# pierrepaleo/PDWT

Hardware: AMD Instinct MI355X
Metric: Mpixels/s fwd+inv DWT (4096² db4 L3) (higher is better)
Workload: dtype f32; 1 GPU; 4096x4096 float32, db4, 3 levels, separable DWT fwd+inv (BASELINE.json configs[1]); levels=3, parallelism=batch-split x1 (no data-path collective)

## Files before the change

### pdwt_amd/csrc/casc_dev.hpp

```cpp
#pragma once
#include "common.hpp"

#ifndef PDWT_CASC_DIAG
#define PDWT_CASC_DIAG 0
#endif
#define CASC_DIAG_ST(row) ((PDWT_CASC_DIAG & 1) ? ((row) & 31) : (row))
#define CASC_DIAG_LD(row) ((PDWT_CASC_DIAG & 2) ? ((row) & 31) : (row))

namespace pdwt {

template <int HLEN>
struct CascGeom {
    static constexpr int C = HLEN / 2 - 1;
    static constexpr int NB1 = C > 0 ? (C + 3) / 4 : 0;
    static constexpr int NB2 = C > 0 ? (C + 1) / 2 : 0;
    static constexpr int NBT = NB1 + NB2;
    static constexpr int WIN1 = 4 * (2 * NB1 + 1);
    static constexpr int WIN2 = 2 * (2 * NB2 + 1);
    static constexpr int MAXVL = 64 - 2 * NBT;
};

struct CascMap {
    int cpx;
    int strips;
// ... 4 lines not shown
__host__ __device__ inline int casc_chunk_start(int g, int strip, int units, int gy, int strips, int cpx, int d)
{
    if (g >= gy) return units;
    int b = (int)(((long long)g * units) / gy);
    if (d != 0) {
        int bal = 0;
        for (int q = 0; q < g; q++) bal += (((q * strips + strip) / cpx) & 1) ? -1 : 1;
        b += d * bal;
    }
    return b;
}

struct CascBands {
    float *H1, *V1, *D1, *A2, *H2, *V2, *D2;
};
struct CascBatchF {
    const float* in;
    CascBands b;
};

template <int HLEN>
struct CascInvGeom {
    static constexpr int H2 = HLEN / 2;
    static constexpr int C = H2 / 2;
    static constexpr int SHIFT = (H2 & 1) ? 0 : 1;
    static constexpr int NB1 = C > 0 ? (C + 1) / 2 : 0;
    static constexpr int NB2 = C;
    static constexpr int NBT = NB1 + NB2;
    static constexpr int WIN1 = 2 * (2 * NB1 + 1);
    static constexpr int WIN2 = 2 * NB2 + 1;
// ... 45 lines not shown
```

### pdwt_amd/csrc/common.hpp

```cpp
#pragma once
#include <atomic>
#include <hip/hip_runtime.h>
#include <hip/hip_ext.h>
#include <stddef.h>
#include <stdint.h>

#include "../../include/pdwt_hip.h"

namespace pdwt {

void set_last_error(hipError_t e, const char* what, const char* file, int line);

#define PDWT_HIP_TRY(expr)                                              \
    do {                                                                \
        hipError_t _e = (expr);                                         \
        if (_e != hipSuccess) {                                         \
            ::pdwt::set_last_error(_e, #expr, __FILE__, __LINE__);      \
            return PDWT_EHIP;                                           \
        }                                                               \
    } while (0)

hipStream_t stream();

enum KernelId {
// ... 126 lines not shown
    KN_F64_LDS_SKEW,
    KN_NORM2SQ_REF1D,
    KN_NORM_IN_THRESHOLD,
    KN_SELFCHECK,
    KN_DWT1D_F64,
    KN_SWTF_LONG,
    KN_F64_TAIL,
    KN_EXP0,
    KN_EXP1,
    KN_EXP2,
    KN_EXP3,
    KN_NONSEP_TILED,
    KN_F64_LAT,
    KN_F64_LAT_MIN,
    KN_DWT1D_NT_MB,
    KN_COUNT
};
int knob(KnobId id);
bool counted_waits_ok();
void stat_casc_spec(int inverse);
enum StatId {
    ST_INV_CASC3,
    ST_INV_CASCW,
    ST_INV_CASC2,
    ST_FWD1D_FUSED,
    ST_INV1D_FUSED,
    ST_FWD1D_FUSED_IP,
    ST_INV1D_FUSED_IP,
    ST_ANA_ROWS_TR,
    ST_SYN_ROWS_TR,
    ST_ANA_COLS_RING,
    ST_SYN_COLS_RING,
    ST_SWT_ANA_ROWS_LDS,
    ST_SWT_SYN_ROWS_LDS,
    ST_SWT_ANA_COLS_RING,
    ST_SWT_SYN_COLS_RING,
    ST_SWTF_FWD,
    ST_SWTF_INV,
    ST_SWTF_INVP,
    ST_SWTL2_FWD,
    ST_SWTL2_INV,
    ST_SWTD_FWD,
    ST_SWTD_INV,
    ST_COUNT
};
void stat_hit(StatId id);
int knob_set(const char* name, int value);
int knob_get(const char* name, int* value);

__host__ __device__ inline int div2(int n) { return (n + 1) >> 1; }
inline int idiv_up(int a, int b) { return (a + b - 1) / b; }

__device__ __forceinline__ int wrap_ext(int s, int n)
{
    const int np = n + (n & 1);
    if ((unsigned)s >= (unsigned)np) {
        s %= np;
        if (s < 0) s += np;
// ... 50 lines not shown
```

### pdwt_amd/csrc/dwt.hip

```cpp
#include <stdlib.h>
#include <string.h>

#include "common.hpp"
#include "cols_ring.hpp"
#include "rows_tr.hpp"
#include "dwt1d_fused.hpp"
#include <new>
#include <vector>

#include "dwt_lds.hpp"
#include "dwt_lat.hpp"
#include "dwt_stream.hpp"
#include "dwt_casc.hpp"
#include "casc_dev.hpp"

namespace pdwt {

constexpr int kThreads = 256;

template <typename T, int HLEN, int TX, int TY>
__global__ __launch_bounds__(kThreads) void k_fwd2d_fused(const T* __restrict__ in, T* __restrict__ cA, T* __restrict__ cH,
                                                           T* __restrict__ cV, T* __restrict__ cD, int Nr, int Nc, int hlen_rt,
                                                           Taps2<T> f)
{
// ... 589 lines not shown
template <typename T>
static int forward_separable(T* d_image, T** c, T* d_tmp, pdwt_info w, const typename FiltersOf<T>::type* filt)
{
    int rc = check_args(d_image, c, d_tmp, w, 2, true, filt, filt ? filt->hlen : 0);
    if (rc != PDWT_OK) return rc;
    const Taps2<T> f = taps_fwd<T>(filt);
    Scratch<T> s(d_tmp, w.Nr, w.Nc, 2);
    const T* in = d_image;
    int nr = w.Nr, nc = w.Nc;
    int pp = 0;
    for (int lev = 0; lev < w.nlevels; lev++) {
        if constexpr (sizeof(T) == 4) {
            if (lev + 1 < w.nlevels && !force_twopass()) {
                T* a2 = (lev + 2 == w.nlevels) ? c[0] : s.ping[pp];
                float* trash = s.t1_is_trash ? (float*)s.t1 : nullptr;
                rc = fwd2d_casc_f32(in, c[3 * lev + 1], c[3 * lev + 2], c[3 * lev + 3], a2, c[3 * lev + 4], c[3 * lev + 5], c[3 * lev + 6],
                                    trash, nr, nc, w.hlen, f);
                if (rc < 0) return rc;
                if (rc == PDWT_OK) {
                    in = a2;
                    pp ^= 1;
                    nr = div2(div2(nr));
                    nc = div2(div2(nc));
                    lev++;
                    continue;
                }
            }
        }
        T* aout = (lev == w.nlevels - 1) ? c[0] : s.ping[pp];
        rc = level_fwd2d(in, aout, c[3 * lev + 1], c[3 * lev + 2], c[3 * lev + 3], s.t1, s.t2, s.trash_floats, nr, nc, w.hlen, f,
                         d_tmp + pdwt_tmp_elems(w) - 256);
        if (rc != PDWT_OK) return rc;
        in = aout;
// ... 562 lines not shown
```

### pdwt_amd/csrc/dwt_casc.hip

```cpp
#include "dwt_casc.hpp"

#include <algorithm>

#include "dwt_stream.hpp"
#include "stream_dev.hpp"
#include "casc_dev.hpp"

namespace pdwt {

constexpr int casc_fwd_stores(int p) { return 3 + 4 * (p & 1); }
template <int DIST>
constexpr int casc_fwd_after(int p)
{
    int n = casc_fwd_stores(p);
    for (int k = 1; k < DIST; k++) n += 2 + casc_fwd_stores(p + k);
    return n;
}

template <int HLEN>
constexpr int casc_fwd_region_bytes() { return (HLEN - 2) * 64 * (16 + 8); }

#define PDWT_VB_F0 " op_sel_hi:[0,1,0]"
#define PDWT_VB_N0 " op_sel_hi:[0,1,1]"
#define PDWT_VB_F1 " op_sel:[1,0,0] op_sel_hi:[1,1,0]"
// ... 49 lines not shown
template <int HLEN, int R2, bool LV, int DIST>
struct CascSpec {
    static constexpr int NA = 2 * R2, NA1 = NA + HLEN - 2, NL1 = NA - HLEN / 2 + 1;
    static constexpr int LIM = LV ? NA1 : NL1;
    static constexpr int stores_at(int q) { return ((q < NA) ? 3 : 0) + (((q & 1) && q >= HLEN - 1) ? 4 : 0); }
    static constexpr int loads_at(int q) { return (q < LIM && q + DIST < LIM) ? 2 : 0; }
    static constexpr int wait_cnt(int n)
    {
        const int m = n - DIST;
        int c = stores_at(m);
        for (int k = 1; k < DIST; k++) c += loads_at(m + k) + stores_at(m + k);
        return c;
    }
};

template <int HLEN, int NV, int W, bool SPEC = false>
__global__ __launch_bounds__(W == 1 ? 256 : 64 * W) void k_fwd2d_casc(const float* in, CascBands b, int Nr, int Nc, int VL,
                                                                       float* __restrict__ trash, CascMap cm, TapsLH f)
{
    using G = CascGeom<HLEN>;
    constexpr int C = G::C, NB1 = G::NB1, NB2 = G::NB2, NBT = G::NBT, WIN1 = G::WIN1, WIN2 = G::WIN2;
    extern __shared__ __attribute__((aligned(16))) unsigned char lds_raw[];
    CASC_TRACE_DECL;
    CASC_TRACE(0);
    if constexpr (W > 1) {
        if (cm.tbl) {
            static_assert(sizeof(CascBatchF) == 8 * sizeof(void*), "eight pointers per image");
            typedef const unsigned long long __attribute__((address_space(4))) * tbl_t;
            const tbl_t q = (tbl_t)(const unsigned long long*)cm.tbl + 8 * (size_t)blockIdx.y;
            in = (const float*)q[0];
            b = CascBands{(float*)q[1], (float*)q[2], (float*)q[3], (float*)q[4], (float*)q[5], (float*)q[6], (float*)q[7]};
        }
    }
// ... 139 lines not shown
            }
            lplast = p1;
        } else {
            p0 = p1 = lplast;
        }
        lr += 2;
    };
    unsigned s1off = (unsigned)wrap1(2 * j0 - C, Nr2) * (unsigned)Nc2 * 4u;
    const unsigned s1end = (unsigned)Nr2 * (unsigned)Nc2 * 4u;
    unsigned s2off = (unsigned)j0 * (unsigned)Nc4 * 4u;
    (void)trash;
    const int hand_sb = __builtin_amdgcn_readfirstlane((W > 1 && kw > 0) ? 0 : -1);
    CASC_TRACE(1);
    static_for<NV>([&](auto K) { asm_drain1(v[decltype(K)::value]); });
    CASC_TRACE(2);
    auto a1_row = [&](auto A, int sb) {
            constexpr int a = decltype(A)::value;
            constexpr int u = a % (HLEN / 2);
            constexpr int s0 = (2 * u + HLEN - 2) % HLEN, s1 = (2 * u + HLEN - 1) % HLEN;
            const int n = sb * HLEN + a;
            constexpr int r0 = (2 * a) % NV, r1 = r0 + 1;
            int nq1 = n, nq2 = n;
            asm("" : "+s"(nq1));
            asm("" : "+s"(nq2));
            if (nq2 < lim2) {
                if (nq1 < lim1) {
                    asm_wait2<casc_fwd_after<DIST>((a + HLEN - DIST) % HLEN)>(v[r0], v[r1]);
                    row_pass1(v[r0], ring[s0]);
                    row_pass1(v[r1], ring[s1]);
                } else {
// ... 36 lines not shown
                    if (sb == hand_sb) *lds_ring2(lds_wr, a) = ring2[a];
                }
            } else {
                if constexpr (W > 1) ring2[a] = *lds_ring2(lds_rd, min(n - NA, HLEN - 3));
            }
            if constexpr (a & 1) {
                v2f ah2 = {0.f, 0.f}, vd2 = {0.f, 0.f};
                static_for<HLEN>([&](auto J) {
                    constexpr int j = decltype(J)::value;
                    constexpr int s = (a + 1 + j) % HLEN;
                    const v2f t = f.t[HLEN - 1 - j];
                    ah2 = pk_fma(splat(ring2[s].x), t, ah2);
                    vd2 = pk_fma(splat(ring2[s].y), t, vd2);
                });
                const bool own = (unsigned)(n - (HLEN - 1)) < (unsigned)(2 * rows2);
                asm_store4_sm(b.A2, b.H2, b.V2, b.D2, off2 + s2off, ah2.x, ah2.y, vd2.x, vd2.y, own ? vmask : 0ull);
                s2off += own ? (unsigned)Nc4 * 4u : 0u;
            }
    };
    auto epilogue = [&]() __attribute__((always_inline)) {
        CASC_TRACE(5);
#ifdef PDWT_CASC_TRACE
        asm volatile("s_waitcnt vmcnt(0)" ::: "memory");
#endif
        CASC_TRACE(6);
        CASC_TRACE_STORE(trash, blockIdx.x * W + kw, ((unsigned long long)NA1 << 32) | (unsigned)rows2);
    };
    if constexpr (SPEC) {
        static_assert(W == 16 && (NV == 2 || NV == 4), "wave programs exist for the 16-wave workgroups");
        const unsigned xoff_odd = xoff + (unsigned)strideB;
        auto spec = [&](auto R2c, auto LASTc) __attribute__((always_inline)) {
            constexpr int R2 = decltype(R2c)::value;
            constexpr bool LV = decltype(LASTc)::value;
            using S = CascSpec<HLEN, R2, LV, DIST>;
            constexpr int sNA = S::NA, sNA1 = S::NA1, sNL1 = S::NL1;
            constexpr int WR = LV ? 4 * R2 + 3 * C : 3 * C;
// ... 72 lines not shown
                if constexpr ((n & 1) && n >= HLEN - 1) {
                    v2f ah2 = {0.f, 0.f}, vd2 = {0.f, 0.f};
                    if constexpr (HLEN == 8) {
                        constexpr int q = (a + 1) % 8;
                        col_pass8x1(ah2, vd2, ring2[q], ring2[(q + 1) % 8], ring2[(q + 2) % 8], ring2[(q + 3) % 8], ring2[(q + 4) % 8], ring2[(q + 5) % 8],
                                    ring2[(q + 6) % 8], ring2[(q + 7) % 8], f.t[7], f.t[6], f.t[5], f.t[4], f.t[3], f.t[2], f.t[1], f.t[0]);
                    } else {
                        static_for<HLEN>([&](auto J) {
                            constexpr int j = decltype(J)::value;
                            constexpr int s = (a + 1 + j) % HLEN;
                            const v2f t = f.t[HLEN - 1 - j];
                            ah2 = pk_fma_vbcast<0, j == 0>(ring2[s], t, ah2);
                            vd2 = pk_fma_vbcast<1, j == 0>(ring2[s], t, vd2);
                        });
                    }
                    asm_store4_sm(b.A2, b.H2, b.V2, b.D2, off2 + s2off, ah2.x, ah2.y, vd2.x, vd2.y, vmask);
                    s2off += (unsigned)Nc4 * 4u;
                }
                if constexpr (n == HLEN / 2 - 1 || n == HLEN - 1) asm volatile("s_waitcnt lgkmcnt(0)\n\ts_barrier" ::: "memory");

#ifdef PDWT_CASC_TRACE
                if constexpr (n == HLEN / 2 - 1) CASC_TRACE(3);
                if constexpr (n == HLEN - 1) CASC_TRACE(4);
#endif
            });
        };
        const int variant = __builtin_amdgcn_readfirstlane(last ? 3 : (rows2 == 5 ? 2 : 1));
        if (variant == 1) {
            spec(std::integral_constant<int, 4>{}, std::false_type{});
            epilogue();
            __builtin_amdgcn_endpgm();
// ... 15 lines not shown
        if (sb == 0) CASC_TRACE(3);
#endif
        if (sb * HLEN + HLEN / 2 >= NA1) break;
        static_for<HLEN / 2>([&](auto U) { a1_row(std::integral_constant<int, decltype(U)::value + HLEN / 2>{}, sb); });
        if constexpr (W > 1) {
            if (sb == 0) asm volatile("s_waitcnt lgkmcnt(0)\n\ts_barrier" ::: "memory");
        }
#ifdef PDWT_CASC_TRACE
        if (sb == 0) CASC_TRACE(4);
#endif
        if (sb * HLEN + HLEN >= NA1) break;
    }
    static_for<NV>([&](auto K) { asm_drain1(v[decltype(K)::value]); });
    epilogue();
    }
}

template <int HLEN, int PFD>
__global__ __launch_bounds__(256) void k_inv2d_casc(CascInvBands b, float* __restrict__ out, int Nr, int Nc, int VL,
                                                     float* __restrict__ trash, CascMap cm, Taps2<float> f)
{
    using G = CascInvGeom<HLEN>;
    constexpr int H2 = G::H2, C = G::C, SHIFT = G::SHIFT, NB1 = G::NB1, NB2 = G::NB2, NBT = G::NBT, WIN1 = G::WIN1, WIN2 = G::WIN2;
    constexpr int VM_PF = PFD * (4 + 2 * (3 + 2));
    static_assert(VM_PF - 3 <= 63, "vmcnt is a 6-bit counter");
    static_assert(H2 % PFD == 0 || PFD % H2 == 0, "register slots must be compile-time constants");
    const int lane = threadIdx.x & 63;
    const int xcd = blockIdx.x & 7;
    const int wi = (blockIdx.x >> 3) * 4 + __builtin_amdgcn_readfirstlane(threadIdx.x >> 6);
    if (wi >= cm.cpx * cm.strips) return;
// ... 242 lines not shown
        asm_drain1(q2[k][2]);
        asm_drain1(q2[k][3]);
    });
    static_for<2 * PFD>([&](auto K) {
        constexpr int k = decltype(K)::value;
        asm_drain1(q1[k][0]);
        asm_drain1(q1[k][1]);
        asm_drain1(q1[k][2]);
    });
}

#define PDWT_CHECK_LAUNCH() PDWT_HIP_TRY(hipGetLastError())

static bool casc_enabled() { return knob(KN_CASC) == 1; }

template <int HLEN>
static int launch_fwd_casc(const float* in, const CascBands& b, float* trash, int nr, int nc, const Taps2<float>& f2, const CascBatchF* d_tbl, int nimg)
{
    TapsLH f;
    for (int k = 0; k < PDWT_MAX_FILTER_WIDTH; k++) f.t[k] = v2f{f2.a[k], f2.b[k]};
    constexpr int MAXVL = CascGeom<HLEN>::MAXVL;
    const int strips = idiv_up(nc, MAXVL * 4);
    const int VL = idiv_up(nc / 4, strips);
    constexpr int NVD = HLEN > 16 ? 4 : (HLEN % 4 == 0 ? HLEN / 2 : HLEN);
    KTimer kt(K_FWD2D_CASC, true);
    int W = knob(KN_CASC_WG);
    if (W == 0) W = 16;
    if (W != 1 && W != 4 && W != 8 && W != 16) W = 16;
    constexpr size_t REG = casc_fwd_region_bytes<HLEN>();
    while (W > 1 && (size_t)(W - 1) * REG > 150 * 1024) W /= 2;
    if (W == 2) W = 1;
    if (W > 1) {
        const int nr4 = nr / 4;
        const int wgs = knob(KN_CASC_WAVES) > 0 ? idiv_up(knob(KN_CASC_WAVES), W) : 256;
        int gy = std::max(1, wgs / strips);
        while (W > 4 && (nr4 / gy) / W < HLEN / 2) W /= 2;
        while (gy > 1 && (nr4 / gy) / W < HLEN / 2) gy--;
        if (gy >= 1 && (nr4 / gy) / W >= HLEN / 2) {
            int nwg = gy * strips;
            const size_t lds = (size_t)(W - 1) * REG;
            void (*k)(const float*, CascBands, int, int, int, float*, CascMap, TapsLH);
            k = (W == 4) ? k_fwd2d_casc<HLEN, NVD, 4> : (W == 8) ? k_fwd2d_casc<HLEN, NVD, 8> : k_fwd2d_casc<HLEN, NVD, 16>;
            const bool nv2 = W == 16 && (knob(KN_CASC_NV) == 0 || knob(KN_CASC_NV) == 2);
            if (nv2) k = k_fwd2d_casc<HLEN, 2, 16>;
            bool spec = nv2 && (knob(KN_CASC_SPEC) & 1) && 2 * 4 >= HLEN;
            auto spec_ok = [&](int gyq, int xwq) {
                const int cpxq = idiv_up(gyq * strips, 8);
                for (int g = 0; g < gyq; g++)
                    for (int st = 0; st < strips; st++) {
                        const int R = casc_chunk_start(g + 1, st, nr4, gyq, strips, cpxq, xwq) - casc_chunk_start(g, st, nr4, gyq, strips, cpxq, xwq);
                        if (R < 16) return false;
                        const int E = std::min((3 * (HLEN - 2) + 3) / 4, R / 16 - 1);
                        const int base = (R + E) / 16, rem = (R + E) % 16;
                        if (base != 4 || R - (15 * base + std::min(15, rem)) != 1) return false;
                    }
                return true;
            };
            if (spec && (knob(KN_CASC_SPEC) & 4) && knob(KN_CASC_WAVES) <= 0 && !d_tbl && (nr4 / gy) / 16 >= 8) {
                const int gy2 = (nr4 + 36) / 73;
                if (gy2 >= 3 * gy && spec_ok(gy2, 0)) {
                    gy = gy2;
                    nwg = gy * strips;
                }
            }
            int xw = spec ? knob(KN_CASC_XCDW) : 0;
            if (spec && xw != 0 && !spec_ok(gy, xw)) xw = 0;
            spec = spec && spec_ok(gy, xw);
            if (!spec) xw = 0;
            if (spec) {
                k = k_fwd2d_casc<HLEN, 2, 16, true>;
                stat_casc_spec(0);
            }
            const CascMap cm = {idiv_up(nwg, 8), strips, gy, xw, d_tbl};
            const dim3 grid((unsigned)(8 * cm.cpx), (unsigned)(d_tbl ? nimg : 1));
            if (lds > 64 * 1024) {
                int rc = (W == 4) ? lds_opt_in<k_fwd2d_casc<HLEN, NVD, 4>>()
                         : (W == 8) ? lds_opt_in<k_fwd2d_casc<HLEN, NVD, 8>>() : lds_opt_in<k_fwd2d_casc<HLEN, NVD, 16>>();
                if (rc == PDWT_OK && nv2) rc = lds_opt_in<k_fwd2d_casc<HLEN, 2, 16>>();
                if (rc == PDWT_OK && spec) rc = lds_opt_in<k_fwd2d_casc<HLEN, 2, 16, true>>();
                if (rc != PDWT_OK) return rc;
            }
            PDWT_LAUNCH_KT(kt, k, grid, dim3(64 * W), lds, in, b, nr, nc, VL, trash, cm, f);
            PDWT_CHECK_LAUNCH();
            return PDWT_OK;
        }
    }
    if (d_tbl) return 1;
    int cpx = (knob(KN_CASC_WAVES) > 0 ? knob(KN_CASC_WAVES) : 1024) / (8 * strips);
    if (cpx > nr / 4 / 4 / 8) cpx = nr / 4 / 4 / 8;
    if (cpx < 1) cpx = 1;
    const CascMap cm = {cpx, strips, 0};
    const dim3 grid((unsigned)(8 * idiv_up(cpx * strips, 4)));
    const int nv = knob(KN_CASC_NV) > 0 ? knob(KN_CASC_NV) : NVD;
    if (nv == 2)
        PDWT_LAUNCH_KT(kt, (k_fwd2d_casc<HLEN, 2, 1>), grid, dim3(256), 0, in, b, nr, nc, VL, trash, cm, f);
    else if (nv < HLEN && HLEN % 4 == 0)
        PDWT_LAUNCH_KT(kt, (k_fwd2d_casc<HLEN, NVD, 1>), grid, dim3(256), 0, in, b, nr, nc, VL, trash, cm, f);
    else
        PDWT_LAUNCH_KT(kt, (k_fwd2d_casc<HLEN, (HLEN > 16 ? NVD : HLEN), 1>), grid, dim3(256), 0, in, b, nr, nc, VL, trash, cm, f);
    PDWT_CHECK_LAUNCH();
    return PDWT_OK;
}

#ifdef PDWT_CASC_ONLY8
#define PDWT_CASC_FWD_HLENS(X) X(8)
#else
#define PDWT_CASC_FWD_HLENS(X) X(4) X(6) X(8) X(10) X(12) X(14) X(16) X(18) X(20)
#endif

int fwd2d_casc_f32(const float* in, float* H1, float* V1, float* D1, float* A2, float* H2, float* V2, float* D2, float* trash, int nr,
                   int nc, int hlen, const Taps2<float>& f, const CascBatchF* d_tbl, int nimg)
{
    if (!casc_enabled() || !stream_enabled() || !trash) return 1;
    if ((nr & 3) || (nc & 3) || nc < 256 || nr < 16 * hlen) return 1;
    if ((long long)nr * nc < (long long)knob(KN_CASC_MIN)) return 1;
    if ((long long)nr * nc >= (1LL << 32)) return 1;
    if (!al16(in) || !al16(H1) || !al16(V1) || !al16(D1) || !al16(A2) || !al16(H2) || !al16(V2) || !al16(D2)) return 1;
    const CascBands b = {H1, V1, D1, A2, H2, V2, D2};
    switch (hlen) {
#define X(H) \
    case H: return launch_fwd_casc<H>(in, b, trash, nr, nc, f, d_tbl, nimg);
        PDWT_CASC_FWD_HLENS(X)
#undef X
        default: return 1;
    }
}

template <int HLEN>
static int launch_inv_casc(const CascInvBands& b, float* out, float* trash, int nr, int nc, const Taps2<float>& f)
{
    constexpr int MAXVL = CascInvGeom<HLEN>::MAXVL;
    const int nc1 = nc / 2;
    const int strips = idiv_up(nc1, MAXVL * 2);
    const int VL = idiv_up(nc1 / 2, strips);
    int cpx = (knob(KN_CASC_IWAVES) > 0 ? knob(KN_CASC_IWAVES) : 2048) / (8 * strips);
    if (cpx > nr / 2 / 8 / 8) cpx = nr / 2 / 8 / 8;
// ... 50 lines not shown
```

### pdwt_amd/csrc/dwt_casc.hpp

```cpp
#pragma once
#include "common.hpp"
#include "casc_dev.hpp"

namespace pdwt {
int fwd2d_casc_f32(const float* in, float* H1, float* V1, float* D1, float* A2, float* H2, float* V2, float* D2, float* trash, int nr,
                   int nc, int hlen, const Taps2<float>& f, const CascBatchF* d_tbl = nullptr, int nimg = 1);
int inv2d_casc_f32(const float* A2, const float* H2, const float* V2, const float* D2, const float* H1, const float* V1, const float* D1,
                   float* out, float* trash, int nr, int nc, int hlen, const Taps2<float>& f);
}
```

### pdwt_amd/csrc/runtime.hip

```cpp
#include <set>
#include <utility>
#include <stdio.h>
#include <stdlib.h>
#include <string.h>

#include <mutex>
#include <vector>

#include "common.hpp"

namespace pdwt {

static thread_local char g_err[512] = "";

void set_last_error(hipError_t e, const char* what, const char* file, int line)
{
    snprintf(g_err, sizeof(g_err), "%s: %s (%s:%d)", hipGetErrorString(e), what, file, line);
    (void)hipGetLastError();
}

static std::mutex g_mu;
static hipStream_t g_streams[64] = {};
static hipStream_t g_user_streams[64] = {};
static bool g_user_set[64] = {};
// ... 30 lines not shown
static const KnobDef g_knob_defs[KN_COUNT] = {
    {"force_twopass", "PDWT_FORCE_TWOPASS", 0}, {"tiled_cols", "PDWT_TILED_COLS", 0},
    {"casc", "PDWT_CASC", 1}, {"casc_waves", "PDWT_CASC_WAVES", 0}, {"casc_nv", "PDWT_CASC_NV", 0},
    {"casc_min", "PDWT_CASC_MIN", 2048 * 2048}, {"casc_iwaves", "PDWT_CASC_IWAVES", 0}, {"casc_ipfd", "PDWT_CASC_IPFD", 1},
    {"casc_wg", "PDWT_CASC_WG", 0}, {"casc_iwg", "PDWT_CASC_IWG", 0}, {"casc_l3", "PDWT_CASC_L3", 1}, {"casc_spec", "PDWT_CASC_SPEC", 7}, {"casc_xcdw", "PDWT_CASC_XCDW", 0}, {"dwt1d_lds_kb", "PDWT_DWT1D_LDS_KB", 80},
    {"stream", "PDWT_STREAM", 1}, {"stream_r", "PDWT_STREAM_R", 0}, {"stream_waves", "PDWT_STREAM_WAVES", 8192},
    {"stream_narrow", "PDWT_STREAM_NARROW", 2048 * 2048}, {"small", "PDWT_SMALL", 1},
    {"rows_tr", "PDWT_ROWS_TR", 1}, {"ring_r", "PDWT_RING_R", 0}, {"ring_waves", "PDWT_RING_WAVES", 4096},
    {"swtf", "PDWT_SWTF", 1}, {"swtf_m", "PDWT_SWTF_M", 0}, {"swtf_mi", "PDWT_SWTF_MI", 0},
    {"swtf_xcd", "PDWT_SWTF_XCD", 1}, {"swtf_alt", "PDWT_SWTF_ALT", 1}, {"swtf_perm", "PDWT_SWTF_PERM", 1}, {"swtf_f64", "PDWT_SWTF_F64", 1},
    {"f64_lds", "PDWT_F64_LDS", 1}, {"f64_lds_min", "PDWT_F64_LDS_MIN", 256}, {"f64_lds_wgs", "PDWT_F64_LDS_WGS", 512}, {"f64_lds_mingroups", "PDWT_F64_LDS_MINGROUPS", 1}, {"f64_lds_skew", "PDWT_F64_LDS_SKEW", 64}, {"norm2sq_ref1d", "PDWT_NORM2SQ_REF1D", 0},
    {"norm_in_threshold", "PDWT_NORM_IN_THRESHOLD", -1},
    {"selfcheck", "PDWT_SELFCHECK", 1}, {"dwt1d_f64", "PDWT_DWT1D_F64", 1}, {"swtf_long", "PDWT_SWTF_LONG", 1}, {"f64_tail", "PDWT_F64_TAIL", 0},
    {"exp0", "PDWT_EXP0", 0}, {"exp1", "PDWT_EXP1", 0}, {"exp2", "PDWT_EXP2", 0}, {"exp3", "PDWT_EXP3", 0}, {"nonsep_tiled", "PDWT_NONSEP_TILED", 1},
    {"f64_lat", "PDWT_F64_LAT", 1}, {"f64_lat_min", "PDWT_F64_LAT_MIN", 4096}, {"dwt1d_nt_mb", "PDWT_DWT1D_NT_MB", 192},
};
static int g_knob_vals[KN_COUNT];
static std::once_flag g_knob_once;
static void knob_init()
{
    for (int i = 0; i < KN_COUNT; i++) {
        const char* e = getenv(g_knob_defs[i].env);
        g_knob_vals[i] = (e && *e) ? atoi(e) : g_knob_defs[i].dflt;
    }
}
int knob(KnobId id)
{
    std::call_once(g_knob_once, knob_init);
    return g_knob_vals[id];
}
// ... 5 lines not shown
        if (!strcmp(name, g_knob_defs[i].name)) {
            g_knob_vals[i] = value;
            return PDWT_OK;
        }
    }
    return PDWT_EINVAL;
}

std::atomic<int> g_stat_spec_fwd{0}, g_stat_spec_inv{0};
void stat_casc_spec(int inverse) { (inverse ? g_stat_spec_inv : g_stat_spec_fwd).fetch_add(1, std::memory_order_relaxed); }
std::atomic<int> g_stat_lat_fwd{0}, g_stat_lat_inv{0};
void stat_lat(int inverse) { (inverse ? g_stat_lat_inv : g_stat_lat_fwd).fetch_add(1, std::memory_order_relaxed); }
static const char* const g_stat_names[ST_COUNT] = {
    "inv_casc3", "inv_cascw", "inv_casc2", "fwd1d_fused", "inv1d_fused", "fwd1d_fused_ip", "inv1d_fused_ip", "ana_rows_tr", "syn_rows_tr",
    "ana_cols_ring", "syn_cols_ring", "swt_ana_rows_lds", "swt_syn_rows_lds", "swt_ana_cols_ring", "swt_syn_cols_ring",
    "swtf_fwd", "swtf_inv", "swtf_invp", "swtl2_fwd", "swtl2_inv", "swtd_fwd", "swtd_inv",
};
static std::atomic<int> g_stat_hits[ST_COUNT];
void stat_hit(StatId id) { g_stat_hits[id].fetch_add(1, std::memory_order_relaxed); }

int knob_get(const char* name, int* value)
{
    std::call_once(g_knob_once, knob_init);
    if (!name || !value) return PDWT_EINVAL;
    if (!strcmp(name, "stat_casc_spec_fwd") || !strcmp(name, "stat_casc_spec_inv")) {
        *value = (name[15] == 'f' ? g_stat_spec_fwd : g_stat_spec_inv).load(std::memory_order_relaxed);
        return PDWT_OK;
    }
    if (!strcmp(name, "stat_lat_fwd") || !strcmp(name, "stat_lat_inv")) {
        *value = (name[9] == 'f' ? g_stat_lat_fwd : g_stat_lat_inv).load(std::memory_order_relaxed);
        return PDWT_OK;
// ... 205 lines not shown
{
    float ms = -1.f;
    if (hipEventElapsedTime(&ms, (hipEvent_t)a, (hipEvent_t)b) != hipSuccess) return -1.f;
    return ms;
}
int pdwt_event_destroy(void* ev)
{
    PDWT_HIP_TRY(hipEventDestroy((hipEvent_t)ev));
    return PDWT_OK;
}

int pdwt_graph_allowed(void) { return (g_kt_on || g_probe_on) ? 0 : 1; }
int pdwt_graph_capture_begin(void)
{
    (void)pdwt::counted_waits_ok();
    PDWT_HIP_TRY(hipStreamBeginCapture(pdwt::stream(), hipStreamCaptureModeThreadLocal));
    return PDWT_OK;
}
int pdwt_graph_capture_end(void** exec_out)
{
    if (!exec_out) return PDWT_EINVAL;
    *exec_out = nullptr;
    hipGraph_t g = nullptr;
    hipError_t e = hipStreamEndCapture(pdwt::stream(), &g);
    if (e != hipSuccess || !g) {
        (void)hipGetLastError();
        return PDWT_EHIP;
    }
    hipGraphExec_t x = nullptr;
    e = hipGraphInstantiate(&x, g, nullptr, nullptr, 0);
// ... 130 lines not shown
```

### pdwt_amd/csrc/stream_dev.hpp

```cpp
#pragma once
#include <stdlib.h>

#include <type_traits>

#include "common.hpp"

#if defined(__HIP_DEVICE_COMPILE__) && !defined(__gfx950__)
#error "pdwt_amd streaming kernels: gfx950 (MI355X) only -- see stream_dev.hpp"
#endif

namespace pdwt {

__device__ __forceinline__ float dpp_shr1(float src)
{
    return __int_as_float(__builtin_amdgcn_mov_dpp(__float_as_int(src), 0x138, 0xf, 0xf, true));
}
__device__ __forceinline__ float dpp_shl1(float src)
{
    return __int_as_float(__builtin_amdgcn_mov_dpp(__float_as_int(src), 0x130, 0xf, 0xf, true));
}

__device__ __forceinline__ int wrapi(int s, int n)
{
    s %= n;
// ... 116 lines not shown
    asm volatile("s_and_saveexec_b64 %0, %4\n\tglobal_store_dwordx4 %1, %2, %3\n\ts_nop 1\n\ts_mov_b64 exec, %0"
                 : "=&s"(saved) : "v"(voff), "v"(d), "s"(sbase), "s"(mask) : "memory", "scc");
}
__device__ __forceinline__ void asm_store3_sm(float* b0, float* b1, float* b2, unsigned voff, v2f d0, v2f d1, v2f d2, lanemask_t mask)
{
    lanemask_t saved;
    asm volatile("s_and_saveexec_b64 %0, %8\n\tglobal_store_dwordx2 %1, %2, %5\n\tglobal_store_dwordx2 %1, %3, %6\n\tglobal_store_dwordx2 %1, %4, %7\n\ts_mov_b64 exec, %0"
                 : "=&s"(saved) : "v"(voff), "v"(d0), "v"(d1), "v"(d2), "s"(b0), "s"(b1), "s"(b2), "s"(mask) : "memory", "scc");
}
__device__ __forceinline__ void asm_store4_sm(float* b0, float* b1, float* b2, float* b3, unsigned voff, float d0, float d1, float d2, float d3, lanemask_t mask)
{
    lanemask_t saved;
    asm volatile("s_and_saveexec_b64 %0, %10\n\tglobal_store_dword %1, %2, %6\n\tglobal_store_dword %1, %3, %7\n\tglobal_store_dword %1, %4, %8\n\tglobal_store_dword %1, %5, %9\n\ts_mov_b64 exec, %0"
                 : "=&s"(saved) : "v"(voff), "v"(d0), "v"(d1), "v"(d2), "v"(d3), "s"(b0), "s"(b1), "s"(b2), "s"(b3), "s"(mask) : "memory", "scc");
}
__device__ __forceinline__ void asm_store_sm_nt(float* sbase, unsigned voff, v4f d, lanemask_t mask)
{
    lanemask_t saved;
    asm volatile("s_and_saveexec_b64 %0, %4\n\tglobal_store_dwordx4 %1, %2, %3 nt\n\ts_nop 1\n\ts_mov_b64 exec, %0"
                 : "=&s"(saved) : "v"(voff), "v"(d), "s"(sbase), "s"(mask) : "memory", "scc");
}
__device__ __forceinline__ float asm_copy(const float& src)
{
    float d;
    asm volatile("v_mov_b32 %0, %1" : "=v"(d) : "v"(src));
    return d;
}
__device__ __forceinline__ v2f asm_copy(const v2f& src)
{
    v2f d;
// ... 38 lines not shown
```

Baseline: 344,200 Mpixels/s.

## Fold third DWT level into cascaded forward kernel via tile completion counters

When the forward cascade kernel produces the second-to-last level, each workgroup now bumps atomic counters for its neighbouring tiles, and the last contributor for a tile computes the third level (A3/H3/V3/D3) from the freshly written A2 in LDS. This removes the separate level-3 kernel launch and the re-read pass over A2. In exchange it adds atomics, acquire fences, extra LDS per workgroup (which may reduce occupancy), and tail work done serially by the last workgroup of each neighbourhood.

```diff
diff --git a/pdwt_amd/csrc/casc_dev.hpp b/pdwt_amd/csrc/casc_dev.hpp
--- a/pdwt_amd/csrc/casc_dev.hpp
+++ b/pdwt_amd/csrc/casc_dev.hpp
@@ -42,6 +42,21 @@
 struct CascBands {
     float *H1, *V1, *D1, *A2, *H2, *V2, *D2;
 };
+struct CascFl3 {
+    float *A3, *H3, *V3, *D3;
+    unsigned* cnt;
+    int need;
+    int flags;
+};
+__host__ __device__ inline int casc_fl3_ring(int n) { return n < 3 ? n : 3; }
+__host__ __device__ inline int casc_fl3_first(int a0) { return (a0 + 1) >> 1; }
+constexpr int kFl3LdsHead = 64 * sizeof(int);
+__host__ __device__ inline size_t casc_fl3_lds(int oy, int ox, int hlen)
+{
+    const size_t ri = 2 * (size_t)oy + hlen - 2, ci = 2 * (size_t)ox + hlen - 2;
+    return kFl3LdsHead + sizeof(float) * (ri * ci + 2 * ri * (size_t)ox);
+}
+
 struct CascBatchF {
     const float* in;
     CascBands b;
diff --git a/pdwt_amd/csrc/common.hpp b/pdwt_amd/csrc/common.hpp
--- a/pdwt_amd/csrc/common.hpp
+++ b/pdwt_amd/csrc/common.hpp
@@ -164,11 +164,13 @@
     KN_F64_LAT,
     KN_F64_LAT_MIN,
     KN_DWT1D_NT_MB,
+    KN_CASC_FL3,
     KN_COUNT
 };
 int knob(KnobId id);
 bool counted_waits_ok();
 void stat_casc_spec(int inverse);
+unsigned* casc_fl3_counters();
 enum StatId {
     ST_INV_CASC3,
     ST_INV_CASCW,
@@ -192,6 +194,7 @@
     ST_SWTL2_INV,
     ST_SWTD_FWD,
     ST_SWTD_INV,
+    ST_CASC_FL3,
     ST_COUNT
 };
 void stat_hit(StatId id);
diff --git a/pdwt_amd/csrc/dwt.hip b/pdwt_amd/csrc/dwt.hip
--- a/pdwt_amd/csrc/dwt.hip
+++ b/pdwt_amd/csrc/dwt.hip
@@ -627,9 +627,13 @@
             if (lev + 1 < w.nlevels && !force_twopass()) {
                 T* a2 = (lev + 2 == w.nlevels) ? c[0] : s.ping[pp];
                 float* trash = s.t1_is_trash ? (float*)s.t1 : nullptr;
+                const bool tail = (lev + 3 == w.nlevels);
+                const CascL3Out b3 = {c[0], tail ? c[3 * lev + 7] : nullptr, tail ? c[3 * lev + 8] : nullptr, tail ? c[3 * lev + 9] : nullptr};
+                bool folded = false;
                 rc = fwd2d_casc_f32(in, c[3 * lev + 1], c[3 * lev + 2], c[3 * lev + 3], a2, c[3 * lev + 4], c[3 * lev + 5], c[3 * lev + 6],
-                                    trash, nr, nc, w.hlen, f);
+                                    trash, nr, nc, w.hlen, f, nullptr, 1, tail ? &b3 : nullptr, &folded);
                 if (rc < 0) return rc;
+                if (rc == PDWT_OK && folded) return PDWT_OK;
                 if (rc == PDWT_OK) {
                     in = a2;
                     pp ^= 1;
diff --git a/pdwt_amd/csrc/dwt_casc.hip b/pdwt_amd/csrc/dwt_casc.hip
--- a/pdwt_amd/csrc/dwt_casc.hip
+++ b/pdwt_amd/csrc/dwt_casc.hip
@@ -1,6 +1,8 @@
 #include "dwt_casc.hpp"
 
 #include <algorithm>
+#include <cstddef>
+#include <mutex>
 
 #include "dwt_stream.hpp"
 #include "stream_dev.hpp"
@@ -87,9 +89,119 @@
     }
 };
 
-template <int HLEN, int NV, int W, bool SPEC = false>
-__global__ __launch_bounds__(W == 1 ? 256 : 64 * W) void k_fwd2d_casc(const float* in, CascBands b, int Nr, int Nc, int VL,
-                                                                       float* __restrict__ trash, CascMap cm, TapsLH f)
+struct CascFwdArgs {
+    const float* in;
+    CascBands b;
+    int Nr, Nc, VL;
+    float* trash;
+    CascMap cm;
+    TapsLH f;
+    CascFl3 fl;
+};
+static_assert(offsetof(CascFwdArgs, b) == 8 && offsetof(CascFwdArgs, Nr) == 64 && offsetof(CascFwdArgs, trash) == 80 && offsetof(CascFwdArgs, cm) == 88 &&
+                  offsetof(CascFwdArgs, f) == 112 && offsetof(CascFwdArgs, fl) == 112 + sizeof(TapsLH) && sizeof(CascFl3) == 48,
+              "the argument offsets in the code object's metadata (llvm-readelf --notes) for k_fwd2d_casc_l3");
+typedef const CascFwdArgs __attribute__((address_space(4))) * casc_fwd_args_t;
+template <int HLEN, int W>
+__device__ __forceinline__ void casc_fl3_finish(unsigned char* lds)
+{
+    constexpr int C = HLEN / 2 - 1;
+    casc_fwd_args_t ka = (casc_fwd_args_t)__builtin_amdgcn_kernarg_segment_ptr();
+    asm volatile("" : "+s"(ka));
+    unsigned* const cnt = ka->fl.cnt;
+    if (!cnt) return;
+    asm volatile("s_waitcnt vmcnt(0) lgkmcnt(0)\n\ts_barrier" ::: "memory");
+    const int lane = threadIdx.x & 63, kw = __builtin_amdgcn_readfirstlane(threadIdx.x >> 6);
+    const CascMap cm = {ka->cm.cpx, ka->cm.strips, ka->cm.gy, ka->cm.flags, nullptr};
+    const int VL = ka->VL, Nr4 = ka->Nr >> 2, Nc4 = ka->Nc >> 2;
+    const float* const A2 = ka->b.A2;
+    const int xflags = ka->fl.flags;
+    const struct { float *A3, *H3, *V3, *D3; int need; } fl = {ka->fl.A3, ka->fl.H3, ka->fl.V3, ka->fl.D3, ka->fl.need};
+    struct { v2f t[HLEN]; } f;
+#pragma unroll
+    for (int j = 0; j < HLEN; j++) f.t[j] = ka->f.t[j];
+    const int wg = (blockIdx.x & 7) * cm.cpx + (blockIdx.x >> 3);
+    const int wgy = wg / cm.strips, strip = wg - wgy * cm.strips;
+    int* const flag = reinterpret_cast<int*>(lds);
+    if (kw == 0) {
+        const int r = min(lane / 3, 2), c = lane % 3;
+        const bool on = lane < 9 && r < casc_fl3_ring(cm.gy) && c < casc_fl3_ring(cm.strips);
+        const int tile = wrap1(wgy + r - 1, cm.gy) * cm.strips + wrap1(strip + c - 1, cm.strips);
+        const unsigned got = asm_ticket_sm(cnt, (unsigned)tile * 4u, __ballot(on));
+        const bool mine = on && got + 1u == (unsigned)fl.need;
+        asm_store_sm_wt(cnt, (unsigned)tile * 4u, 0u, __ballot(mine));
+        flag[lane] = mine ? tile : -1;
+    }
+    __syncthreads();
+    const int Nc8 = Nc4 >> 1;
+    float* const win = reinterpret_cast<float*>(lds + kFl3LdsHead);
+    for (int k = 0; k < 9; k++) {
+        const int tile = __builtin_amdgcn_readfirstlane(flag[k]);
+        if (tile < 0 || (xflags & 2)) continue;
+        if (!(xflags & 1)) __builtin_amdgcn_fence(__ATOMIC_ACQUIRE, "agent");
+        const int tg = tile / cm.strips, ts = tile - tg * cm.strips;
+        const int J0 = casc_chunk_start(tg, ts, Nr4, cm.gy, cm.strips, cm.cpx, cm.flags);
+        const int J1 = casc_chunk_start(tg + 1, ts, Nr4, cm.gy, cm.strips, cm.cpx, cm.flags);
+        const int X0 = ts * VL, X1 = min(X0 + VL, Nc4);
+        const int oy0 = casc_fl3_first(J0), OY = casc_fl3_first(J1) - oy0, ox0 = casc_fl3_first(X0), OX = casc_fl3_first(X1) - ox0;
+        const int RI = 2 * OY + HLEN - 2, CI = 2 * OX + HLEN - 2;
+        float* const rb = win + RI * CI;
+        {
+            const int gy0 = 2 * oy0 - C, gx0 = 2 * ox0 - C;
+            const int c0 = min(lane, CI - 1), c1 = min(lane + 64, CI - 1);
+            const int gc0 = wrapi(gx0 + c0, Nc4), gc1 = wrapi(gx0 + c1, Nc4);
+            for (int r = kw; r < RI; r += 4 * W) {
+                float v0[4], v1[4];
+#pragma unroll
+                for (int u = 0; u < 4; u++) {
+                    const float* const row = A2 + (size_t)wrapi(gy0 + min(r + u * W, RI - 1), Nr4) * Nc4;
+                    v0[u] = __hip_atomic_load(row + gc0, __ATOMIC_RELAXED, __HIP_MEMORY_SCOPE_AGENT);
+                    v1[u] = __hip_atomic_load(row + gc1, __ATOMIC_RELAXED, __HIP_MEMORY_SCOPE_AGENT);
+                }
+#pragma unroll
+                for (int u = 0; u < 4; u++) {
+                    const int rr = min(r + u * W, RI - 1);
+                    win[rr * CI + c0] = v0[u];
+                    win[rr * CI + c1] = v1[u];
+                }
+            }
+        }
+        __syncthreads();
+        const int ox = min(lane & 31, OX - 1), half = lane >> 5;
+        for (int r0 = 2 * kw; r0 < RI; r0 += 2 * W) {
+            const int r = r0 + half;
+            const float* const p = win + r * CI + 2 * ox;
+            float lo = 0.f, hi = 0.f;
+#pragma unroll
+            for (int j = 0; j < HLEN; j++) {
+                const float v = p[j];
+                lo = __builtin_fmaf(v, f.t[HLEN - 1 - j].x, lo);
+                hi = __builtin_fmaf(v, f.t[HLEN - 1 - j].y, hi);
+            }
+            rb[r * OX + ox] = lo;
+            rb[(RI + r) * OX + ox] = hi;
+        }
+        __syncthreads();
+        float* const b0 = half ? fl.V3 : fl.A3;
+        float* const b1 = half ? fl.D3 : fl.H3;
+        for (int oy = kw; oy < OY; oy += W) {
+            const float* const p = rb + (half * RI + 2 * oy) * OX + ox;
+            float lo = 0.f, hi = 0.f;
+#pragma unroll
+            for (int j = 0; j < HLEN; j++) {
+                const float v = p[j * OX];
+                lo = __builtin_fmaf(v, f.t[HLEN - 1 - j].x, lo);
+                hi = __builtin_fmaf(v, f.t[HLEN - 1 - j].y, hi);
+            }
+            const size_t o = (size_t)(oy0 + oy) * Nc8 + (ox0 + ox);
+            b0[o] = lo;
+            b1[o] = hi;
+        }
+    }
+}
+
+template <int HLEN, int NV, int W, bool SPEC, bool FL3>
+__device__ __forceinline__ void casc_fwd_body(const float* in, CascBands b, int Nr, int Nc, int VL, float* __restrict__ trash, CascMap cm, TapsLH f)
 {
     using G = CascGeom<HLEN>;
     constexpr int C = G::C, NB1 = G::NB1, NB2 = G::NB2, NBT = G::NBT, WIN1 = G::WIN1, WIN2 = G::WIN2;
@@ -259,6 +371,10 @@
     CASC_TRACE(1);
     static_for<NV>([&](auto K) { asm_drain1(v[decltype(K)::value]); });
     CASC_TRACE(2);
+    auto store_l2 = [&](unsigned voff, float a, float h, float vv, float d, lanemask_t m) __attribute__((always_inline)) {
+        if constexpr (FL3) asm_store4_sm_wt0(b.A2, b.H2, b.V2, b.D2, voff, a, h, vv, d, m);
+        else asm_store4_sm(b.A2, b.H2, b.V2, b.D2, voff, a, h, vv, d, m);
+    };
     auto a1_row = [&](auto A, int sb) {
             constexpr int a = decltype(A)::value;
             constexpr int u = a % (HLEN / 2);
@@ -325,12 +441,15 @@
                     vd2 = pk_fma(splat(ring2[s].y), t, vd2);
                 });
                 const bool own = (unsigned)(n - (HLEN - 1)) < (unsigned)(2 * rows2);
-                asm_store4_sm(b.A2, b.H2, b.V2, b.D2, off2 + s2off, ah2.x, ah2.y, vd2.x, vd2.y, own ? vmask : 0ull);
+                store_l2(off2 + s2off, ah2.x, ah2.y, vd2.x, vd2.y, own ? vmask : 0ull);
                 s2off += own ? (unsigned)Nc4 * 4u : 0u;
             }
     };
     auto epilogue = [&]() __attribute__((always_inline)) {
         CASC_TRACE(5);
+        if constexpr (FL3) {
+            casc_fl3_finish<HLEN, W>(lds_raw);
+        }
 #ifdef PDWT_CASC_TRACE
         asm volatile("s_waitcnt vmcnt(0)" ::: "memory");
 #endif
@@ -433,7 +552,7 @@
                             vd2 = pk_fma_vbcast<1, j == 0>(ring2[s], t, vd2);
                         });
                     }
-                    asm_store4_sm(b.A2, b.H2, b.V2, b.D2, off2 + s2off, ah2.x, ah2.y, vd2.x, vd2.y, vmask);
+                    store_l2(off2 + s2off, ah2.x, ah2.y, vd2.x, vd2.y, vmask);
                     s2off += (unsigned)Nc4 * 4u;
                 }
                 if constexpr (n == HLEN / 2 - 1 || n == HLEN - 1) asm volatile("s_waitcnt lgkmcnt(0)\n\ts_barrier" ::: "memory");
@@ -479,6 +598,20 @@
     static_for<NV>([&](auto K) { asm_drain1(v[decltype(K)::value]); });
     epilogue();
     }
+}
+
+template <int HLEN, int NV, int W, bool SPEC = false>
+__global__ __launch_bounds__(W == 1 ? 256 : 64 * W) void k_fwd2d_casc(const float* in, CascBands b, int Nr, int Nc, int VL,
+                                                                       float* __restrict__ trash, CascMap cm, TapsLH f)
+{
+    casc_fwd_body<HLEN, NV, W, SPEC, false>(in, b, Nr, Nc, VL, trash, cm, f);
+}
+template <int HLEN, int NV, int W, bool SPEC = false>
+__global__ __launch_bounds__(64 * W) void k_fwd2d_casc_l3(const float* in, CascBands b, int Nr, int Nc, int VL, float* __restrict__ trash, CascMap cm,
+                                                          TapsLH f, CascFl3 fl)
+{
+    (void)fl;
+    casc_fwd_body<HLEN, NV, W, SPEC, true>(in, b, Nr, Nc, VL, trash, cm, f);
 }
 
 template <int HLEN, int PFD>
@@ -751,8 +884,33 @@
 
 static bool casc_enabled() { return knob(KN_CASC) == 1; }
 
+constexpr int kFl3MaxTiles = 16384;
+static std::mutex g_fl3_mu;
+static unsigned* g_fl3_cnt[64] = {};
+unsigned* casc_fl3_counters()
+{
+    int dev = 0;
+    if (hipGetDevice(&dev) != hipSuccess || dev < 0 || dev >= 64) return nullptr;
+    std::lock_guard<std::mutex> lk(g_fl3_mu);
+    if (!g_fl3_cnt[dev]) {
+        hipStreamCaptureStatus cs = hipStreamCaptureStatusNone;
+        if (hipStreamIsCapturing(stream(), &cs) != hipSuccess || cs != hipStreamCaptureStatusNone) {
+            (void)hipGetLastError();
+            return nullptr;
+        }
+        if (hipMalloc(&g_fl3_cnt[dev], kFl3MaxTiles * sizeof(unsigned)) != hipSuccess) g_fl3_cnt[dev] = nullptr;
+        else if (hipMemsetAsync(g_fl3_cnt[dev], 0, kFl3MaxTiles * sizeof(unsigned), stream()) != hipSuccess) {
+            (void)hipFree(g_fl3_cnt[dev]);
+            g_fl3_cnt[dev] = nullptr;
+        }
+        if (!g_fl3_cnt[dev]) (void)hipGetLastError();
+    }
+    return g_fl3_cnt[dev];
+}
+
 template <int HLEN>
-static int launch_fwd_casc(const float* in, const CascBands& b, float* trash, int nr, int nc, const Taps2<float>& f2, const CascBatchF* d_tbl, int nimg)
+static int launch_fwd_casc(const float* in, const CascBands& b, float* trash, int nr, int nc, const Taps2<float>& f2, const CascBatchF* d_tbl, int nimg,
+                           const CascL3Out* b3, bool* folded)
 {
     TapsLH f;
     for (int k = 0; k < PDWT_MAX_FILTER_WIDTH; k++) f.t[k] = v2f{f2.a[k], f2.b[k]};
@@ -775,11 +933,13 @@
         while (gy > 1 && (nr4 / gy) / W < HLEN / 2) gy--;
         if (gy >= 1 && (nr4 / gy) / W >= HLEN / 2) {
             int nwg = gy * strips;
-            const size_t lds = (size_t)(W - 1) * REG;
+            size_t lds = (size_t)(W - 1) * REG;
             void (*k)(const float*, CascBands, int, int, int, float*, CascMap, TapsLH);
             k = (W == 4) ? k_fwd2d_casc<HLEN, NVD, 4> : (W == 8) ? k_fwd2d_casc<HLEN, NVD, 8> : k_fwd2d_casc<HLEN, NVD, 16>;
+            void (*k3)(const float*, CascBands, int, int, int, float*, CascMap, TapsLH, CascFl3);
+            k3 = (W == 4) ? k_fwd2d_casc_l3<HLEN, NVD, 4> : (W == 8) ? k_fwd2d_casc_l3<HLEN, NVD, 8> : k_fwd2d_casc_l3<HLEN, NVD, 16>;
             const bool nv2 = W == 16 && (knob(KN_CASC_NV) == 0 || knob(KN_CASC_NV) == 2);
-            if (nv2) k = k_fwd2d_casc<HLEN, 2, 16>;
+            if (nv2) k = k_fwd2d_casc<HLEN, 2, 16>, k3 = k_fwd2d_casc_l3<HLEN, 2, 16>;
             bool spec = nv2 && (knob(KN_CASC_SPEC) & 1) && 2 * 4 >= HLEN;
             auto spec_ok = [&](int gyq, int xwq) {
                 const int cpxq = idiv_up(gyq * strips, 8);
@@ -806,10 +966,32 @@
             if (!spec) xw = 0;
             if (spec) {
                 k = k_fwd2d_casc<HLEN, 2, 16, true>;
+                k3 = k_fwd2d_casc_l3<HLEN, 2, 16, true>;
                 stat_casc_spec(0);
             }
             const CascMap cm = {idiv_up(nwg, 8), strips, gy, xw, d_tbl};
             const dim3 grid((unsigned)(8 * cm.cpx), (unsigned)(d_tbl ? nimg : 1));
+            CascFl3 fl = {nullptr, nullptr, nullptr, nullptr, nullptr, 0, 0};
+            if (b3 && !d_tbl && knob(KN_CASC_FL3) == 1 && !(nr4 & 1) && !((nc / 4) & 1) && nwg <= kFl3MaxTiles) {
+                constexpr int C = HLEN / 2 - 1;
+                const int nc4 = nc / 4;
+                bool ok = VL >= C + 1 && nc4 - (strips - 1) * VL >= C + 1;
+                size_t need = 0;
+                for (int g = 0; g < gy && ok; g++)
+                    for (int st = 0; st < strips; st++) {
+                        const int J0 = casc_chunk_start(g, st, nr4, gy, strips, cm.cpx, xw), J1 = casc_chunk_start(g + 1, st, nr4, gy, strips, cm.cpx, xw);
+                        const int X0 = st * VL, X1 = std::min(X0 + VL, nc4);
+                        if (J1 - J0 < C + 1) ok = false;
+                        need = std::max(need, casc_fl3_lds(casc_fl3_first(J1) - casc_fl3_first(J0), casc_fl3_first(X1) - casc_fl3_first(X0), HLEN));
+                    }
+                unsigned* const cnt = (ok && need <= 150 * 1024) ? casc_fl3_counters() : nullptr;
+                if (cnt) {
+                    fl = CascFl3{b3->A3, b3->H3, b3->V3, b3->D3, cnt, casc_fl3_ring(gy) * casc_fl3_ring(strips), knob(KN_EXP0)};
+                    lds = std::max(lds, need);
+                    stat_hit(ST_CASC_FL3);
+                    *folded = true;
+                }
+            }
             if (lds > 64 * 1024) {
                 int rc = (W == 4) ? lds_opt_in<k_fwd2d_casc<HLEN, NVD, 4>>()
                          : (W == 8) ? lds_opt_in<k_fwd2d_casc<HLEN, NVD, 8>>() : lds_opt_in<k_fwd2d_casc<HLEN, NVD, 16>>();
@@ -817,7 +999,13 @@
                 if (rc == PDWT_OK && spec) rc = lds_opt_in<k_fwd2d_casc<HLEN, 2, 16, true>>();
                 if (rc != PDWT_OK) return rc;
             }
-            PDWT_LAUNCH_KT(kt, k, grid, dim3(64 * W), lds, in, b, nr, nc, VL, trash, cm, f);
+            if (fl.cnt) {
+                if (lds > 64 * 1024)
+                    if (const int rc = lds_opt_in_ptr((const void*)k3); rc != PDWT_OK) return rc;
+                PDWT_LAUNCH_KT(kt, k3, grid, dim3(64 * W), lds, in, b, nr, nc, VL, trash, cm, f, fl);
+            } else {
+                PDWT_LAUNCH_KT(kt, k, grid, dim3(64 * W), lds, in, b, nr, nc, VL, trash, cm, f);
+            }
             PDWT_CHECK_LAUNCH();
             return PDWT_OK;
         }
@@ -846,8 +1034,10 @@
 #endif
 
 int fwd2d_casc_f32(const float* in, float* H1, float* V1, float* D1, float* A2, float* H2, float* V2, float* D2, float* trash, int nr,
-                   int nc, int hlen, const Taps2<float>& f, const CascBatchF* d_tbl, int nimg)
-{
+                   int nc, int hlen, const Taps2<float>& f, const CascBatchF* d_tbl, int nimg, const CascL3Out* b3, bool* folded)
+{
+    if (folded) *folded = false;
+    if (b3 && (!folded || !b3->A3 || !al16(b3->A3) || !al16(b3->H3) || !al16(b3->V3) || !al16(b3->D3))) b3 = nullptr;
     if (!casc_enabled() || !stream_enabled() || !trash) return 1;
     if ((nr & 3) || (nc & 3) || nc < 256 || nr < 16 * hlen) return 1;
     if ((long long)nr * nc < (long long)knob(KN_CASC_MIN)) return 1;
@@ -856,7 +1046,7 @@
     const CascBands b = {H1, V1, D1, A2, H2, V2, D2};
     switch (hlen) {
 #define X(H) \
-    case H: return launch_fwd_casc<H>(in, b, trash, nr, nc, f, d_tbl, nimg);
+    case H: return launch_fwd_casc<H>(in, b, trash, nr, nc, f, d_tbl, nimg, b3, folded);
         PDWT_CASC_FWD_HLENS(X)
 #undef X
         default: return 1;
diff --git a/pdwt_amd/csrc/dwt_casc.hpp b/pdwt_amd/csrc/dwt_casc.hpp
--- a/pdwt_amd/csrc/dwt_casc.hpp
+++ b/pdwt_amd/csrc/dwt_casc.hpp
@@ -3,8 +3,12 @@
 #include "casc_dev.hpp"
 
 namespace pdwt {
+struct CascL3Out {
+    float *A3, *H3, *V3, *D3;
+};
 int fwd2d_casc_f32(const float* in, float* H1, float* V1, float* D1, float* A2, float* H2, float* V2, float* D2, float* trash, int nr,
-                   int nc, int hlen, const Taps2<float>& f, const CascBatchF* d_tbl = nullptr, int nimg = 1);
+                   int nc, int hlen, const Taps2<float>& f, const CascBatchF* d_tbl = nullptr, int nimg = 1, const CascL3Out* b3 = nullptr,
+                   bool* folded = nullptr);
 int inv2d_casc_f32(const float* A2, const float* H2, const float* V2, const float* D2, const float* H1, const float* V1, const float* D1,
                    float* out, float* trash, int nr, int nc, int hlen, const Taps2<float>& f);
 }
diff --git a/pdwt_amd/csrc/runtime.hip b/pdwt_amd/csrc/runtime.hip
--- a/pdwt_amd/csrc/runtime.hip
+++ b/pdwt_amd/csrc/runtime.hip
@@ -68,6 +68,7 @@
     {"selfcheck", "PDWT_SELFCHECK", 1}, {"dwt1d_f64", "PDWT_DWT1D_F64", 1}, {"swtf_long", "PDWT_SWTF_LONG", 1}, {"f64_tail", "PDWT_F64_TAIL", 0},
     {"exp0", "PDWT_EXP0", 0}, {"exp1", "PDWT_EXP1", 0}, {"exp2", "PDWT_EXP2", 0}, {"exp3", "PDWT_EXP3", 0}, {"nonsep_tiled", "PDWT_NONSEP_TILED", 1},
     {"f64_lat", "PDWT_F64_LAT", 1}, {"f64_lat_min", "PDWT_F64_LAT_MIN", 4096}, {"dwt1d_nt_mb", "PDWT_DWT1D_NT_MB", 192},
+    {"casc_fl3", "PDWT_CASC_FL3", 1},
 };
 static int g_knob_vals[KN_COUNT];
 static std::once_flag g_knob_once;
@@ -103,7 +104,7 @@
 static const char* const g_stat_names[ST_COUNT] = {
     "inv_casc3", "inv_cascw", "inv_casc2", "fwd1d_fused", "inv1d_fused", "fwd1d_fused_ip", "inv1d_fused_ip", "ana_rows_tr", "syn_rows_tr",
     "ana_cols_ring", "syn_cols_ring", "swt_ana_rows_lds", "swt_syn_rows_lds", "swt_ana_cols_ring", "swt_syn_cols_ring",
-    "swtf_fwd", "swtf_inv", "swtf_invp", "swtl2_fwd", "swtl2_inv", "swtd_fwd", "swtd_inv",
+    "swtf_fwd", "swtf_inv", "swtf_invp", "swtl2_fwd", "swtl2_inv", "swtd_fwd", "swtd_inv", "casc_fl3",
 };
 static std::atomic<int> g_stat_hits[ST_COUNT];
 void stat_hit(StatId id) { g_stat_hits[id].fetch_add(1, std::memory_order_relaxed); }
@@ -339,6 +340,7 @@
 int pdwt_graph_capture_begin(void)
 {
     (void)pdwt::counted_waits_ok();
+    (void)pdwt::casc_fl3_counters();
     PDWT_HIP_TRY(hipStreamBeginCapture(pdwt::stream(), hipStreamCaptureModeThreadLocal));
     return PDWT_OK;
 }
diff --git a/pdwt_amd/csrc/stream_dev.hpp b/pdwt_amd/csrc/stream_dev.hpp
--- a/pdwt_amd/csrc/stream_dev.hpp
+++ b/pdwt_amd/csrc/stream_dev.hpp
@@ -154,6 +154,26 @@
     asm volatile("s_and_saveexec_b64 %0, %10\n\tglobal_store_dword %1, %2, %6\n\tglobal_store_dword %1, %3, %7\n\tglobal_store_dword %1, %4, %8\n\tglobal_store_dword %1, %5, %9\n\ts_mov_b64 exec, %0"
                  : "=&s"(saved) : "v"(voff), "v"(d0), "v"(d1), "v"(d2), "v"(d3), "s"(b0), "s"(b1), "s"(b2), "s"(b3), "s"(mask) : "memory", "scc");
 }
+__device__ __forceinline__ void asm_store4_sm_wt0(float* b0, float* b1, float* b2, float* b3, unsigned voff, float d0, float d1, float d2, float d3, lanemask_t mask)
+{
+    lanemask_t saved;
+    asm volatile("s_and_saveexec_b64 %0, %10\n\tglobal_store_dword %1, %2, %6 sc1\n\tglobal_store_dword %1, %3, %7\n\tglobal_store_dword %1, %4, %8\n\tglobal_store_dword %1, %5, %9\n\ts_mov_b64 exec, %0"
+                 : "=&s"(saved) : "v"(voff), "v"(d0), "v"(d1), "v"(d2), "v"(d3), "s"(b0), "s"(b1), "s"(b2), "s"(b3), "s"(mask) : "memory", "scc");
+}
+__device__ __forceinline__ unsigned asm_ticket_sm(unsigned* sbase, unsigned voff, lanemask_t mask)
+{
+    lanemask_t saved;
+    unsigned got = 0;
+    asm volatile("s_and_saveexec_b64 %0, %5\n\tglobal_atomic_add %1, %2, %3, %4 sc0\n\ts_mov_b64 exec, %0\n\ts_waitcnt vmcnt(0)"
+                 : "=&s"(saved), "+v"(got) : "v"(voff), "v"(1u), "s"(sbase), "s"(mask) : "memory", "scc");
+    return got;
+}
+__device__ __forceinline__ void asm_store_sm_wt(unsigned* sbase, unsigned voff, unsigned d, lanemask_t mask)
+{
+    lanemask_t saved;
+    asm volatile("s_and_saveexec_b64 %0, %4\n\tglobal_store_dword %1, %2, %3 sc1\n\ts_mov_b64 exec, %0"
+                 : "=&s"(saved) : "v"(voff), "v"(d), "s"(sbase), "s"(mask) : "memory", "scc");
+}
 __device__ __forceinline__ void asm_store_sm_nt(float* sbase, unsigned voff, v4f d, lanemask_t mask)
 {
     lanemask_t saved;
```

Result: slower. 141,000 Mpixels/s (-59.0%).
